# Ritesh622/Unbiased-Quantization-Distributed-Mean-Estimation

Hardware: AMD Instinct MI355X
Metric: quantize+dequantize M-vectors/sec at d=2^20 (1/2/4/8 GPU) + NMSE vs reference (higher is better)
Workload: dtype f32

## Files before the change

### include/uq_dme.h

```cpp
#ifndef UQ_DME_H
#define UQ_DME_H

#include <stddef.h>
#include <stdint.h>

#ifdef __cplusplus
extern "C" {
#endif

#define UQ_OK 0
#define UQ_E_INVALID (-1)
#define UQ_E_HIP (-2)
#define UQ_E_WORKSPACE (-3)
#define UQ_E_TIMEOUT (-4)

int uq_version(void);
const char* uq_build_id(void);
int uq_test_force_replay_failure(int on);
int uq_test_set_quicfl_hooks(int flags);
#define UQ_QFL_PLAN_FIELDS 6
#define UQ_QFL_SENDER 0
#define UQ_QFL_RECEIVER 1
#define UQ_QFL_FORM_NONE 0
#define UQ_QFL_FORM_ONE_WAVE 1
// ... 32 lines not shown
int uq_test_last_biased_plan(int64_t* plan_out, int32_t cap);
#define UQ_EDEN_PLAN_FIELDS 25
#define UQ_EDEN_NBITS_FRAC 12
#define UQ_EDEN_MAX_PASSES 4
#define UQ_EDEN_OP_COMPRESS 0
#define UQ_EDEN_OP_DECOMPRESS 1
#define UQ_EDEN_OP_RHT_FORWARD 2
#define UQ_EDEN_OP_RHT_INVERSE 3
#define UQ_EDEN_OP_NORM 4
#define UQ_EDEN_OP_QFL_FRONT 5
#define UQ_EDEN_OP_QFL_INVERSE 6
#define UQ_EDEN_OPS 7
#define UQ_EDEN_NORM_NONE 0
#define UQ_EDEN_NORM_CHAINS_WHOLE 1
#define UQ_EDEN_NORM_CHAINS_GENERIC 2
#define UQ_EDEN_NORM_SEGMENTED 3
#define UQ_EDEN_NORM_FUSED 4
#define UQ_EDEN_DOT_NONE 0
#define UQ_EDEN_DOT_ONE_WAVE 1
#define UQ_EDEN_DOT_SEGMENTED 2
#define UQ_EDEN_DOT_FUSED_REDO 3
#define UQ_EDEN_PASS_LOW16K 1
#define UQ_EDEN_PASS_LOW4096 2
#define UQ_EDEN_PASS_HIGH256 3
#define UQ_EDEN_PASS_SMALL 4
#define UQ_EDEN_PASS_GENERIC 5
int uq_test_eden_plan(int32_t op, int64_t n, int64_t dim, int32_t nbits, int32_t mode, int64_t* plan_out, int32_t cap);
int uq_test_last_eden_plan(int32_t op, int64_t* plan_out, int32_t cap);
#define UQ_EDEN_PACKED_PLAN_FIELDS 4
#define UQ_EDEN_PACKED_NONE 0
#define UQ_EDEN_PACKED_FUSED 1
#define UQ_EDEN_PACKED_CONVERTER 2
int uq_test_set_eden_hooks(int flags);
int uq_test_eden_packed_plan(int32_t op, int64_t n, int64_t dim, int32_t kind, int64_t* plan_out, int32_t cap);
int uq_test_last_eden_packed_plan(int32_t op, int64_t* plan_out, int32_t cap);
int uq_mt_jump_host(const uint32_t* state624, int64_t blocks, uint32_t* out624);

int uq_legacy_draw_f32(uint32_t* key624, int32_t* pos, int32_t* has_gauss, double* gauss, int32_t dist,
                       double a, double b, int64_t n, int64_t d, float* out, double* norm2, int32_t threads);
int uq_legacy_test_params(int64_t min_chunk, int64_t overlap, int64_t* waves, int64_t* misses);

const char* uq_last_error(void);

int uq_rate_to_m(double bits_per_dimension, int64_t d, int64_t* m_out);

int uq_workspace_bytes(int64_t n, int64_t d, int32_t torch_threads, size_t* bytes_out);

int uq_l1_torch_order_f32(const float* x, int64_t n, int64_t d, int32_t torch_threads,
                          float* l1_out, void* ws, size_t ws_bytes, void* stream);

int uq_type_unbiased_f32(const float* x, float* out, int64_t n, int64_t d, int64_t m,
                         const float* X, const float* l1, float* l1_out,
                         int32_t torch_threads, void* ws, size_t ws_bytes, void* stream);

int uq_type_unbiased_vec_f32(const float* x, float* out, int64_t d, int64_t m, float X, int32_t torch_threads,
                             void* ws, size_t ws_bytes, void* stream);

int uq_client_mean_f32(const float* q, int64_t n, int64_t d, int64_t ld, float n_div,
                       int32_t accumulate, float* est, void* stream);

int uq_type_unbiased_mean_f32(const float* x, float* out, int64_t n, int64_t d, int64_t m,
                              const float* X, const float* l1, int32_t torch_threads,
                              float n_div, int32_t accumulate, float* est,
                              void* ws, size_t ws_bytes, void* stream);

int uq_type_unbiased_codes_f32(const float* x, float* out, int8_t* codes, int32_t* kmax,
                               int64_t n, int64_t d, int64_t m, const float* X, const float* l1,
                               float* l1_out, int32_t torch_threads, void* ws, size_t ws_bytes,
                               void* stream);

int uq_type_unbiased_codes_ld_f32(const float* x, float* out, int64_t ldq, int8_t* codes, int64_t ldc,
                                  int32_t* kmax, int64_t n, int64_t d, int64_t m, const float* X,
                                  const float* l1, float* l1_out, int32_t torch_threads, void* ws,
                                  size_t ws_bytes, void* stream);

int uq_type_unbiased_nibbles_ld_f32(const float* x, float* out, int64_t ldq, uint8_t* nib, int64_t ldn,
                                    int32_t* kmax, int64_t n, int64_t d, int64_t m, const float* X,
                                    const float* l1, float* l1_out, int32_t torch_threads, void* ws,
                                    size_t ws_bytes, void* stream);

int uq_nibbles_q_mean_ld_f32(const uint8_t* nib, int64_t ldn, const float* q, int64_t ldq, const float* l1,
                             const int32_t* kmax, int64_t n, int64_t d, int64_t m, float n_div,
                             int32_t accumulate, float* est, void* stream);

int uq_codes_decode_f32(const int8_t* codes, const float* l1, int64_t n, int64_t d, int64_t m,
                        float* out, void* stream);

int uq_codes_mean_f32(const int8_t* codes, const float* l1, const int32_t* kmax, int64_t n, int64_t d,
                      int64_t m, float n_div, int32_t accumulate, float* est, void* stream);

int uq_codes_q_mean_f32(const int8_t* codes, const float* q, int64_t ldq, const float* l1, const int32_t* kmax,
                        int64_t n, int64_t d, int64_t m, float n_div, int32_t accumulate, float* est,
                        void* stream);

int uq_codes_q_mean_ld_f32(const int8_t* codes, int64_t ldc, const float* q, int64_t ldq, const float* l1,
                           const int32_t* kmax, int64_t n, int64_t d, int64_t m, float n_div,
                           int32_t accumulate, float* est, void* stream);

#define UQ_FORM_UNBIASED 0
#define UQ_FORM_BIASED 1
int uq_codes_decode_form_f32(const int8_t* codes, const float* l1, int64_t n, int64_t d, int64_t m, int32_t form,
                             float* out, void* stream);
int uq_codes_mean_form_f32(const int8_t* codes, int64_t ldc, const float* q, int64_t ldq, const float* l1,
                           const int32_t* kmax, int64_t n, int64_t d, int64_t m, int32_t form, float n_div,
                           int32_t accumulate, float* est, void* stream);

#define UQ_TC_EXACT_ZERO_SIGNS 1
#define UQ_TC_BIASED_FORM 2
int uq_tc_bound(int64_t d, size_t* bytes_out);
int uq_tc_workspace_bytes(int64_t n, int64_t d, size_t* bytes_out);
int uq_tc_encode(const int8_t* codes, const float* l1, int64_t n, int64_t d, int64_t m, int32_t flags,
                 uint8_t* msgs, size_t msgs_bytes, uint64_t* offsets, void* ws, size_t ws_bytes, void* stream);
int uq_tc_decode(const uint8_t* msgs, size_t msgs_bytes, const uint64_t* offsets, int64_t n, int64_t d, int64_t m,
                 int8_t* codes, float* l1, int32_t* kmax, int32_t* status, void* stream);

#define UQ_TIES_TORCH 0
#define UQ_TIES_LOWEST_INDEX 1
#define UQ_TIES_HOST_CHECK 4
int uq_biased_workspace_bytes(int64_t n, int64_t d, int32_t torch_threads, size_t* bytes_out);
int uq_type_biased_f32(const float* x, float* out, int64_t n, int64_t d, int64_t m,
                       int32_t torch_threads, int32_t tie_policy, float* l1_out, int32_t* info,
                       void* ws, size_t ws_bytes, void* stream);

int uq_biased_codes_workspace_bytes(int64_t n, int64_t d, int32_t torch_threads, size_t* bytes_out);
int uq_type_biased_codes_f32(const float* x, float* out, int8_t* codes, int32_t* kmax, int64_t n, int64_t d,
                             int64_t m, int32_t torch_threads, int32_t tie_policy, float* l1_out, int32_t* info,
                             void* ws, size_t ws_bytes, void* stream);

int uq_rht_signs(const int32_t* seeds, int64_t rows, int64_t D, int8_t* signs, void* stream);
int uq_rht_f32(const float* x, float* out, int64_t n, int64_t dim, int32_t inverse, const int8_t* signs,
               const int32_t* sign_row, void* ws, size_t ws_bytes, void* stream);
int uq_quicfl_prepare_f32(const int32_t* X, int64_t n, int64_t D, const float* recv_table, int32_t table_rows,
                          int32_t h_len, const int32_t* prng_seeds, const uint8_t* exact_mask, const float* exact_vals,
                          const float* scale, float* out, void* stream);
#define UQ_QFL_BAD_EXACT 32
int uq_quicfl_receive_f32(const void* X, int32_t x_kind, int64_t n, int64_t D, const float* recv_table,
                          int32_t table_rows, int32_t h_len, const int32_t* prng_seeds, const uint8_t* exact_mask,
                          const float* exact_vals, int32_t exact_layout, const int32_t* exact_count, const float* scale,
                          float* out, int32_t* info, void* stream);
int uq_quicfl_receive_workspace_bytes(int64_t n, int64_t D, size_t* bytes_out);
int uq_quicfl_receive_ws_f32(const void* X, int32_t x_kind, int64_t n, int64_t D, const float* recv_table,
                             int32_t table_rows, int32_t h_len, const int32_t* prng_seeds, const uint8_t* exact_mask,
                             const float* exact_vals, int32_t exact_layout, const int32_t* exact_count,
                             const float* scale, float* out, int32_t* info, void* ws, size_t ws_bytes, void* stream);

#define UQ_QFL_BAD_P 1
#define UQ_QFL_BAD_INDEX 2
#define UQ_QFL_BAD_PX 4
#define UQ_QFL_X_RANGE 8
#define UQ_QFL_TIMEOUT 16
#define UQ_QFL_STATE_WORDS 626
int uq_quicfl_workspace_bytes(int64_t n, int64_t dim, size_t* bytes_out);
int uq_quicfl_compress_f32(const float* x, int64_t n, int64_t dim, const int8_t* signs, const int32_t* sign_row,
                           const float* table_xp, const uint32_t* table_packed, int64_t table_numel, int32_t h_len,
                           float delta,
                           const int32_t* prng_seeds, const uint32_t* px_state, const int32_t* px_seeds,
                           uint32_t* px_state_out, void* X, int32_t x_kind, uint8_t* exact_mask, float* exact_vals,
                           int32_t* exact_count, float* scale, int32_t* info, void* ws, size_t ws_bytes, void* stream);
#define UQ_QFL_RECV_INDEX 64
int uq_quicfl_quantize_f32(const float* x, int64_t n, int64_t dim, const int8_t* signs, const int32_t* sign_row,
                           const float* table_xp, const uint32_t* table_packed, int64_t table_numel, int32_t h_len,
                           float delta, const float* recv_table, int32_t recv_numel, const int32_t* prng_seeds,
                           const uint32_t* px_state, const int32_t* px_seeds, uint32_t* px_state_out, float* out,
                           float* scale, int32_t* info, void* ws, size_t ws_bytes, void* stream);
int uq_test_set_quicfl_packed_hooks(int flags);
int uq_test_last_quicfl_packed_plan(int32_t side, int64_t* plan_out, int32_t cap);
// ... 101 lines not shown
```

### unbiased-quantization-distributed-mean-estimation_amd/_lib.py

```python
from __future__ import annotations

import ctypes
import os
import threading

from . import build_ext

_lock = threading.Lock()
_lib = None

_i32, _i64, _f32, _f64, _p, _sz = (ctypes.c_int32, ctypes.c_int64, ctypes.c_float,
                                   ctypes.c_double, ctypes.c_void_p, ctypes.c_size_t)
SIGNATURES = {
    "uq_version": (ctypes.c_int, []),
    "uq_last_error": (ctypes.c_char_p, []),
    "uq_build_id": (ctypes.c_char_p, []),
    "uq_test_force_replay_failure": (ctypes.c_int, [ctypes.c_int]),
    "uq_test_set_quicfl_hooks": (ctypes.c_int, [ctypes.c_int]),
    "uq_test_quicfl_plan": (ctypes.c_int, [_i32, _i64, _i64, _i32, _i32, _p, _i32]),
    "uq_test_last_quicfl_plan": (ctypes.c_int, [_i32, _p, _i32]),
    "uq_test_unbiased_plan": (ctypes.c_int, [_i64, _i64, _i64, _i64, _i32, _i32, _i32, _i32, _i32, _i32, _i32, _i32, _p,
                                             _i32]),
    "uq_test_last_unbiased_plan": (ctypes.c_int, [_p, _i32]),
    "uq_test_biased_plan": (ctypes.c_int, [_i64, _i64, _i32, _i32, _i32, _p, _i32]),
    "uq_test_last_biased_plan": (ctypes.c_int, [_p, _i32]),
    "uq_test_eden_plan": (ctypes.c_int, [_i32, _i64, _i64, _i32, _i32, _p, _i32]),
    "uq_test_last_eden_plan": (ctypes.c_int, [_i32, _p, _i32]),
    "uq_mt_jump_host": (ctypes.c_int, [_p, _i64, _p]),
    "uq_legacy_draw_f32": (ctypes.c_int, [_p, _p, _p, _p, _i32, _f64, _f64, _i64, _i64, _p, _p, _i32]),
    "uq_legacy_test_params": (ctypes.c_int, [_i64, _i64, _p, _p]),
    "uq_rate_to_m": (ctypes.c_int, [_f64, _i64, ctypes.POINTER(_i64)]),
    "uq_workspace_bytes": (ctypes.c_int, [_i64, _i64, _i32, ctypes.POINTER(_sz)]),
    "uq_l1_torch_order_f32": (ctypes.c_int, [_p, _i64, _i64, _i32, _p, _p, _sz, _p]),
    "uq_type_unbiased_f32": (ctypes.c_int, [_p, _p, _i64, _i64, _i64, _p, _p, _p, _i32, _p, _sz, _p]),
    "uq_type_unbiased_vec_f32": (ctypes.c_int, [_p, _p, _i64, _i64, _f32, _i32, _p, _sz, _p]),
    "uq_client_mean_f32": (ctypes.c_int, [_p, _i64, _i64, _i64, _f32, _i32, _p, _p]),
    "uq_type_unbiased_mean_f32": (ctypes.c_int, [_p, _p, _i64, _i64, _i64, _p, _p, _i32, _f32, _i32, _p,
                                                 _p, _sz, _p]),
    "uq_check_status": (ctypes.c_int, [_p, _p]),
    "uq_type_unbiased_codes_f32": (ctypes.c_int, [_p, _p, _p, _p, _i64, _i64, _i64, _p, _p, _p, _i32, _p, _sz, _p]),
    "uq_codes_decode_f32": (ctypes.c_int, [_p, _p, _i64, _i64, _i64, _p, _p]),
    "uq_codes_mean_f32": (ctypes.c_int, [_p, _p, _p, _i64, _i64, _i64, _f32, _i32, _p, _p]),
    "uq_codes_q_mean_f32": (ctypes.c_int, [_p, _p, _i64, _p, _p, _i64, _i64, _i64, _f32, _i32, _p, _p]),
    "uq_type_unbiased_codes_ld_f32": (ctypes.c_int, [_p, _p, _i64, _p, _i64, _p, _i64, _i64, _i64, _p, _p, _p, _i32,
                                                     _p, _sz, _p]),
    "uq_codes_q_mean_ld_f32": (ctypes.c_int, [_p, _i64, _p, _i64, _p, _p, _i64, _i64, _i64, _f32, _i32, _p, _p]),
    "uq_type_unbiased_nibbles_ld_f32": (ctypes.c_int, [_p, _p, _i64, _p, _i64, _p, _i64, _i64, _i64, _p, _p, _p, _i32,
                                                       _p, _sz, _p]),
    "uq_nibbles_q_mean_ld_f32": (ctypes.c_int, [_p, _i64, _p, _i64, _p, _p, _i64, _i64, _i64, _f32, _i32, _p, _p]),
    "uq_codes_decode_form_f32": (ctypes.c_int, [_p, _p, _i64, _i64, _i64, _i32, _p, _p]),
    "uq_codes_mean_form_f32": (ctypes.c_int, [_p, _i64, _p, _i64, _p, _p, _i64, _i64, _i64, _i32, _f32, _i32, _p, _p]),
    "uq_biased_codes_workspace_bytes": (ctypes.c_int, [_i64, _i64, _i32, ctypes.POINTER(_sz)]),
    "uq_type_biased_codes_f32": (ctypes.c_int, [_p, _p, _p, _p, _i64, _i64, _i64, _i32, _i32, _p, _p, _p, _sz, _p]),
    "uq_biased_workspace_bytes": (ctypes.c_int, [_i64, _i64, _i32, ctypes.POINTER(_sz)]),
    "uq_type_biased_f32": (ctypes.c_int, [_p, _p, _i64, _i64, _i64, _i32, _i32, _p, _p, _p, _sz, _p]),
    "uq_rht_signs": (ctypes.c_int, [_p, _i64, _i64, _p, _p]),
    "uq_rht_f32": (ctypes.c_int, [_p, _p, _i64, _i64, _i32, _p, _p, _p, _sz, _p]),
    "uq_quicfl_prepare_f32": (ctypes.c_int, [_p, _i64, _i64, _p, _i32, _i32, _p, _p, _p, _p, _p, _p]),
    "uq_quicfl_receive_f32": (ctypes.c_int, [_p, _i32, _i64, _i64, _p, _i32, _i32, _p, _p, _p, _i32, _p, _p, _p, _p, _p]),
    "uq_quicfl_receive_workspace_bytes": (ctypes.c_int, [_i64, _i64, ctypes.POINTER(_sz)]),
    "uq_quicfl_receive_ws_f32": (ctypes.c_int, [_p, _i32, _i64, _i64, _p, _i32, _i32, _p, _p, _p, _i32, _p, _p, _p, _p,
                                                _p, _sz, _p]),
    "uq_quicfl_workspace_bytes": (ctypes.c_int, [_i64, _i64, ctypes.POINTER(_sz)]),
    "uq_quicfl_quantize_f32": (ctypes.c_int, [_p, _i64, _i64, _p, _p, _p, _p, _i64, _i32, _f32, _p, _i32, _p, _p, _p, _p,
                                              _p, _p, _p, _p, _sz, _p]),
    "uq_quicfl_compress_f32": (ctypes.c_int, [_p, _i64, _i64, _p, _p, _p, _p, _i64, _i32, _f32, _p, _p, _p, _p, _p, _i32,
                                              _p, _p, _p, _p, _p, _p, _sz, _p]),
    "uq_test_set_quicfl_packed_hooks": (ctypes.c_int, [ctypes.c_int]),
    "uq_test_last_quicfl_packed_plan": (ctypes.c_int, [_i32, _p, _i32]),
    "uq_quicfl_packed_words": (ctypes.c_int, [_i64, _i32, ctypes.POINTER(_i64)]),
    "uq_quicfl_pack_x": (ctypes.c_int, [_p, _i32, _i64, _i64, _i32, _p, _p, _p, _p, _p, _p, _p]),
    "uq_quicfl_unpack_x": (ctypes.c_int, [_p, _i64, _i64, _i32, _p, _p, _p, _p, _p, _p]),
    "uq_quicfl_packed_workspace_bytes": (ctypes.c_int, [_i64, _i64, ctypes.POINTER(_sz)]),
    "uq_quicfl_compress_packed_f32": (ctypes.c_int, [_p, _i64, _i64, _p, _p, _p, _p, _i64, _i32, _f32, _p, _p, _p, _p, _p,
                                                     _i32, _p, _p, _p, _p, _p, _p, _p, _sz, _p]),
    "uq_quicfl_receive_packed_workspace_bytes": (ctypes.c_int, [_i64, _i64, ctypes.POINTER(_sz)]),
    "uq_quicfl_receive_packed_f32": (ctypes.c_int, [_p, _i32, _i64, _i64, _p, _i32, _i32, _p, _p, _p, _p, _p, _p, _p, _p,
                                                    _sz, _p]),
    "uq_xxh64": (ctypes.c_uint64, [ctypes.c_char_p, _sz, ctypes.c_uint64]),
    "uq_eden_workspace_bytes": (ctypes.c_int, [_i64, _i64, ctypes.POINTER(_sz)]),
    "uq_eden_compress_f32": (ctypes.c_int, [_p, _i64, _i64, _i32, _p, _p, _p, _p, _p, _sz, _p]),
    "uq_eden_decompress_f32": (ctypes.c_int, [_p, _p, _i64, _i64, _i32, _p, _p, _p, _p, _sz, _p]),
    "uq_eden_f32": (ctypes.c_int, [_p, _p, _i64, _i64, _i32, _p, _p, _p, _p, _sz, _p]),
    "uq_rht_sign_bits": (ctypes.c_int, [_p, _i64, _i64, _p, _p]),
    "uq_eden_compress_f32_sb": (ctypes.c_int, [_p, _i64, _i64, _i32, _p, _p, _p, _p, _p, _p, _sz, _p]),
    "uq_eden_decompress_f32_sb": (ctypes.c_int, [_p, _p, _i64, _i64, _i32, _p, _p, _p, _p, _p, _sz, _p]),
    "uq_eden_f32_sb": (ctypes.c_int, [_p, _p, _i64, _i64, _i32, _p, _p, _p, _p, _p, _sz, _p]),
    "uq_eden_mask_bits": (ctypes.c_int, [_p, _i64, _i64, ctypes.c_uint32, _p, _p]),
    "uq_eden_compress_frac_f32": (ctypes.c_int, [_p, _i64, _i64, _p, _p, _p, _p, _p, _p, _p, _p, _sz, _p]),
    "uq_eden_decompress_frac_f32": (ctypes.c_int, [_p, _p, _i64, _i64, _p, _p, _p, _p, _p, _p, _p, _sz, _p]),
    "uq_eden_frac_f32": (ctypes.c_int, [_p, _p, _i64, _i64, _p, _p, _p, _p, _p, _p, _p, _sz, _p]),
    "uq_test_set_eden_hooks": (ctypes.c_int, [ctypes.c_int]),
    "uq_test_eden_packed_plan": (ctypes.c_int, [_i32, _i64, _i64, _i32, _p, _i32]),
    "uq_test_last_eden_packed_plan": (ctypes.c_int, [_i32, _p, _i32]),
    "uq_eden_packed_words": (ctypes.c_int, [_i64, _i32, ctypes.POINTER(_i64)]),
    "uq_eden_packed_workspace_bytes": (ctypes.c_int, [_i64, _i64, _i32, ctypes.POINTER(_sz)]),
    "uq_eden_mask_ranks": (ctypes.c_int, [_p, _i64, _i64, _p, _p]),
    "uq_eden_pack_bins": (ctypes.c_int, [_p, _i64, _i64, _i32, _p, _p, _p, _p, _p, _p]),
    "uq_eden_unpack_bins": (ctypes.c_int, [_p, _i64, _i64, _i32, _p, _p, _p, _p, _p]),
    "uq_eden_compress_packed_f32": (ctypes.c_int, [_p, _i64, _i64, _i32, _p, _p, _p, _p, _p, _p, _p, _p, _p, _p, _sz, _p]),
    "uq_eden_decompress_packed_f32": (ctypes.c_int, [_p, _p, _i64, _i64, _i32, _p, _p, _p, _p, _p, _p, _p, _p, _sz, _p]),
    "uq_eden_norm_workspace_bytes": (ctypes.c_int, [_i64, _i64, ctypes.POINTER(_sz)]),
    "uq_eden_norm_f32": (ctypes.c_int, [_p, _i64, _i64, _i32, _p, _p, _sz, _p]),
    "uq_rand_workspace_bytes": (ctypes.c_int, [_i64, _i64, ctypes.POINTER(_sz)]),
    "uq_drive_words": (ctypes.c_int, [_i64, ctypes.POINTER(_i64)]),
    "uq_scalar_quantize_f32": (ctypes.c_int, [_p, _p, _i64, _i64, _f32, _p, _p, _p, _p, _p, _sz, _p]),
    "uq_drive_hadamard_f32": (ctypes.c_int, [_p, _p, _i64, _i64, _p, _p, _p, _p, _p, _sz, _p]),
    "uq_kashin_padded_dim": (ctypes.c_int, [_i64, ctypes.POINTER(_i64)]),
    "uq_kashin_workspace_bytes": (ctypes.c_int, [_i64, _i64, ctypes.POINTER(_sz)]),
    "uq_kashin_compress_f32": (ctypes.c_int, [_p, _i64, _i64, _i64, _i32, _f64, _f64, _f64, _i32, _p, _p, _p, _p, _i64,
                                              _p, _p, _p, _p, _p, _p, _sz, _p]),
    "uq_kashin_decompress_f32": (ctypes.c_int, [_p, _p, _p, _i64, _i64, _i64, _p, _p, _p, _p, _sz, _p]),
    "uq_kashin_f32": (ctypes.c_int, [_p, _p, _i64, _i64, _i64, _i32, _f64, _f64, _f64, _i32, _p, _p, _p, _p, _i64, _p, _p,
                                     _p, _p, _p, _sz, _p]),
    "uq_tc_bound":(ctypes.c_int, [_i64, ctypes.POINTER(_sz)]),
    "uq_tc_workspace_bytes": (ctypes.c_int, [_i64, _i64, ctypes.POINTER(_sz)]),
    "uq_tc_encode": (ctypes.c_int, [_p, _p, _i64, _i64, _i64, _i32, _p, _sz, _p, _p, _sz, _p]),
    "uq_tc_decode": (ctypes.c_int, [_p, _sz, _p, _i64, _i64, _i64, _p, _p, _p, _p, _p]),
}


class UQError(RuntimeError):
    """A C-ABI call returned a negative code."""


def library_path() -> str:
    return build_ext.SO


def load(build_if_missing: bool = False):
    global _lib
    with _lock:
# ... 25 lines not shown
```

### unbiased-quantization-distributed-mean-estimation_amd/csrc/uq_unbiased.hip

```cpp
#include <hip/hip_runtime.h>

#include <algorithm>
#include <cstdint>
#include <type_traits>

#include "uq_internal.h"
#include "uq_unbiased_kernels.h"

namespace {

struct WsLayout {
    size_t agg_off, incl_off, map1_off, rec_off, cnt_off, part_off, l1_off, total;
    int32_t tiles;
    template <class T>
    T* at(void* ws, size_t off) const { return (T*)((char*)ws + off); }
    uint64_t* tile_row(void* ws, size_t off, int64_t j0) const { return at<uint64_t>(ws, off) + j0 * tiles; }
};

WsLayout layout(int64_t n, int64_t d, const L1Plan& plan) {
    WsLayout w{};
    const int64_t tiles = (d + kQTile - 1) / kQTile;
    w.tiles = (int32_t)tiles;
    w.agg_off = kCtrlBytes;
    w.incl_off = up256(w.agg_off + (size_t)n * tiles * sizeof(uint64_t));
    w.map1_off = up256(w.incl_off + (size_t)n * tiles * sizeof(uint64_t));
    const size_t rec_clients = (size_t)std::min<int64_t>(n, kRecClients);
    w.rec_off = up256(w.map1_off + (size_t)n * tiles * sizeof(uint64_t));
    w.cnt_off = up256(w.rec_off + rec_clients * kRecPerClient * sizeof(TileRec));
    w.part_off = up256(w.cnt_off + rec_clients * sizeof(uint32_t));
    w.l1_off = up256(w.part_off + (size_t)n * plan.total_groups * 32 * sizeof(float));
    w.total = up256(w.l1_off + (size_t)n * sizeof(float));
    return w;
}

int launch_l1(const float* x, int64_t n, int64_t d, const L1Plan& plan, float* part, float* l1_out,
              hipStream_t st) {
    return launch_cascade<AbsOp>(x, n, d, plan, part, l1_out, nullptr, 0.f, st);
}

int stream_slots(int* out) {
    int dev = 0;
    int rc = hip_check(hipGetDevice(&dev), "hipGetDevice");
    if (rc) return rc;
    static thread_local int cache_dev = -1, cache_slots = 0;
    if (cache_dev != dev) {
        int cus = 0;
        rc = hip_check(hipDeviceGetAttribute(&cus, hipDeviceAttributeMultiprocessorCount, dev), "CU count");
        if (rc) return rc;
        cache_slots = 4 * std::max(1, cus);
        cache_dev = dev;
    }
    *out = cache_slots;
    return UQ_OK;
}

int check_common(const void* x, int64_t n, int64_t d, int32_t T, void* ws, size_t ws_bytes,
                 L1Plan* plan, WsLayout* w) {
    if (n < 0 || d < 0) return fail(UQ_E_INVALID, "n and d must be >= 0");
    if (n > (int64_t)1 << 31 || d > (int64_t)1 << 40) return fail(UQ_E_INVALID, "n or d too large");
    if (T < 1) return fail(UQ_E_INVALID, "torch_threads must be >= 1");
    if (!make_plan(d, T, plan)) return fail(UQ_E_INVALID, "torch_threads > 4096 (or d too large) unsupported by the L1 plan");
    *w = layout(n, d, *plan);
    if ((int64_t)w->tiles * n > 0xFFFFFFFFll) return fail(UQ_E_INVALID, "batch too large for one call");
    if (n > 0 && d > 0) {
        if (!x) return fail(UQ_E_INVALID, "null input pointer");
        if (!ws) return fail(UQ_E_INVALID, "null workspace");
        if (ws_bytes < w->total) return fail(UQ_E_WORKSPACE, "workspace too small");
    }
    return UQ_OK;
}

}

int uq_internal::launch_l1(const float* x, int64_t n, int64_t d, int32_t T, float* part, float* l1_out,
                           hipStream_t st) {
    L1Plan plan;
    if (!make_plan(d, T, &plan)) return fail(UQ_E_INVALID, "cannot build L1 plan");
    return ::launch_l1(x, n, d, plan, part, l1_out, st);
}

extern "C" {

int uq_workspace_bytes(int64_t n, int64_t d, int32_t T, size_t* bytes_out) {
    if (!bytes_out) return fail(UQ_E_INVALID, "null bytes_out");
    L1Plan plan;
// ... 57 lines not shown
    int32_t prefixed, R, nseg;
};
struct UnbiasedPlan {
    int32_t form;
    bool V, Q, C, CV, l1_given;
    int64_t chunks;
    ChunkPlan last;
    int32_t tiles;
    size_t agg_off, map0_off, map1_off, rec_off, cnt_off;
};

int chunk_plan(const PlanIn& in, const UnbiasedPlan& p, int64_t j0, ChunkPlan* c) {
    c->nj = std::min<int64_t>(kMaxGridY, in.n - j0);
    const int64_t total_tiles = c->nj * (int64_t)p.tiles;
    c->seg = p.V && in.d <= ((int64_t)1 << 29) && total_tiles >= kSegMinTiles;
    c->R = 1;
    c->nseg = 1;
    if (c->seg) {
        int slots = in.slots;
        if (slots <= 0) {
            const int rc = stream_slots(&slots);
            if (rc) return rc;
        }
        const int64_t segs = std::max<int64_t>(1, slots / c->nj);
        c->R = (int32_t)((p.tiles + segs - 1) / segs);
        c->nseg = (p.tiles + c->R - 1) / c->R;
    }
    c->prefixed = c->nj >= 4 ? 1 : 0;
    return UQ_OK;
}

int plan_unbiased(const PlanIn& in, const WsLayout& w, UnbiasedPlan* p) {
    *p = UnbiasedPlan{};
    if (!in.has_out && !in.has_codes) return fail(UQ_E_INVALID, "nothing to write: out and codes are both NULL");
    const int64_t n = in.n, d = in.d;
    p->tiles = w.tiles;
    p->agg_off = w.agg_off;
    p->map0_off = w.incl_off;
    p->map1_off = w.map1_off;
    p->rec_off = w.rec_off;
    p->cnt_off = w.cnt_off;
    p->Q = in.has_out;
    p->C = in.has_codes;
    p->l1_given = in.l1_given;
    p->V = in.x16 && (!in.has_out || in.out16) && ((d % 4 == 0 && in.ldo % 4 == 0) || n == 1);
    p->CV = !in.has_codes || (in.codes16 && d % 16 == 0 && (in.ldc % 16 == 0 || n == 1));
    p->chunks = 1;
    p->last = ChunkPlan{n, false, 0, w.tiles, 1};
    if (!in.nib && d <= kSmallL1Max && p->V && n <= 0x7FFFFFFF) {
        p->form = UQ_FORM_SMALL;
        return UQ_OK;
    }
    const bool stream_form = n >= kStreamMinClients && p->V && d <= ((int64_t)1 << 29);
    if (in.nib) {
        if (!stream_form || !in.has_out || !in.has_codes)
            return fail(UQ_E_INVALID, "internal: 4-bit codes outside the stream form");
        p->form = UQ_FORM_STREAM_NIBBLES;
        p->CV = true;
        return UQ_OK;
    }
    if (stream_form) {
        p->form = UQ_FORM_STREAM;
        return UQ_OK;
    }
    p->chunks = (n + kMaxGridY - 1) / kMaxGridY;
    const int rc = chunk_plan(in, *p, (p->chunks - 1) * kMaxGridY, &p->last);
    if (rc) return rc;
    p->form = p->last.seg ? UQ_FORM_SEGMENTS : UQ_FORM_PHASED;
    return UQ_OK;
}

bool bad_pitches(bool has_out, int64_t ldo, bool has_codes, int64_t ldc, int64_t d, bool nib) {
    return (has_out && ldo < d) || (has_codes && ldc < (nib ? d / 2 : d));
}

bool bad_nibble_shape(int64_t n, int64_t d) {
    return n < kStreamMinClients || d % kNibAlign != 0 || d > ((int64_t)1 << 29);
}
int nibble_shape_error() {
    return fail(UQ_E_INVALID, "4-bit codes need n >= 256 and d a multiple of 4096 (<= 2^29)");
}

thread_local UnbiasedPlan t_last_plan{};

int export_plan(const UnbiasedPlan& p, int64_t* out, int32_t cap) {
    if (!out || cap < 0) return fail(UQ_E_INVALID, "null plan output");
    const int64_t f[UQ_PLAN_FIELDS] = {
        p.form, p.V, p.Q, p.C, p.CV, p.l1_given, p.chunks, p.last.nj, p.last.prefixed, p.last.R, p.last.nseg,
        p.tiles, (int64_t)p.agg_off, (int64_t)p.map0_off, (int64_t)p.map1_off, (int64_t)p.rec_off, (int64_t)p.cnt_off,
        (int64_t)sizeof(TileRec), kRecPerClient, kRecClients, kRecEvents, kFoldEvents};
    for (int i = 0; i < std::min<int32_t>(cap, UQ_PLAN_FIELDS); ++i) out[i] = f[i];
    return UQ_OK;
}

int unbiased_codes_impl(const float* x, float* out, int64_t ldo, int8_t* codes, int64_t ldc, int32_t* overflow,
                        int64_t n, int64_t d, int64_t m, const float* X, float Xval, const float* l1, float* l1_out,
                        int32_t T, void* ws, size_t ws_bytes, void* stream, bool nib = false) {
    L1Plan plan;
    WsLayout w;
    int rc = check_common(x, n, d, T, ws, ws_bytes, &plan, &w);
    if (rc) return rc;
    t_last_plan = UnbiasedPlan{};
    if (m < 0) return fail(UQ_E_INVALID, "m must be >= 0");
    if (bad_pitches(out, ldo, codes, ldc, d, nib)) return fail(UQ_E_INVALID, "row pitches must be >= d");
    if (n == 0 || d == 0) return UQ_OK;
    if (!X && n != 1) return fail(UQ_E_INVALID, "null X");
    const PlanIn in{n, d, ldo, ldc, aligned16(x), aligned16(out), aligned16(codes), out != nullptr, codes != nullptr,
                    nib, l1 != nullptr, 0};
    UnbiasedPlan P;
    rc = plan_unbiased(in, w, &P);
    if (rc) return rc;
    if (codes && !overflow) return fail(UQ_E_INVALID, "codes need a kmax[n] array");
    t_last_plan = P;
    hipStream_t st = (hipStream_t)stream;
    const float* l1use = l1;
    const float fm = (float)m;
    const bool vec4 = P.V, cvec = P.CV;
    if (P.form == UQ_FORM_SMALL) {
        if (!select_qc(out, codes, cvec, [&](auto Q, auto C, auto CV) {
                hipLaunchKernelGGL((quantize_small_kernel<Q(), C(), CV()>), dim3((unsigned)n), dim3(kQBlock), 0, st, x,
                                   out, codes, overflow, d, w.tiles, fm, X, Xval, l1, l1_out, ldo, ldc);
            }))
            return bad_selector();
        return hip_check(hipGetLastError(), "quantize_small_kernel launch");
    }
    if (!l1use) {
        float* l1buf = w.at<float>(ws, w.l1_off);
        rc = launch_l1(x, n, d, plan, w.at<float>(ws, w.part_off), l1buf, st);
        if (rc) return rc;
        l1use = l1buf;
    }
    if (l1_out && l1_out != l1use) {
        rc = hip_check(hipMemcpyAsync(l1_out, l1use, n * sizeof(float), hipMemcpyDeviceToDevice, st), "copy l1");
        if (rc) return rc;
    }
    const bool stream_form = P.form == UQ_FORM_STREAM || P.form == UQ_FORM_STREAM_NIBBLES;
    if (codes && !stream_form) {
        rc = hip_check(hipMemsetAsync(overflow, 0, n * sizeof(int32_t), st), "memset kmax");
        if (rc) return rc;
    }
    if (P.form == UQ_FORM_STREAM_NIBBLES) {
        hipLaunchKernelGGL((quantize_stream_kernel<true, true, true, true>), dim3((unsigned)n), dim3(kQBlock), 0, st, x,
                           out, codes, overflow, d, w.tiles, fm, X, Xval, l1use, w.tiles, 1, nullptr, ldo, ldc);
        return hip_check(hipGetLastError(), "quantize_stream_kernel (4-bit codes) launch");
    }
    if (P.form == UQ_FORM_STREAM) {
        if (!select_qc(out, codes, cvec, [&](auto Q, auto C, auto CV) {
                hipLaunchKernelGGL((quantize_stream_kernel<Q(), C(), CV()>), dim3((unsigned)n), dim3(kQBlock), 0, st, x,
                                   out, codes, overflow, d, w.tiles, fm, X, Xval, l1use, w.tiles, 1, nullptr, ldo, ldc);
            }))
            return bad_selector();
        return hip_check(hipGetLastError(), "quantize_stream_kernel launch");
    }
    for (int64_t j0 = 0; j0 < n; j0 += kMaxGridY) {
        ChunkPlan ck;
        rc = chunk_plan(in, P, j0, &ck);
        if (rc) return rc;
        const int64_t nj = ck.nj;
        const float* xj = x + j0 * d;
        float* outj = out ? out + j0 * ldo : nullptr;
        int8_t* codesj = codes ? codes + j0 * ldc : nullptr;
        int32_t* ovj = codes ? overflow + j0 : nullptr;
        const float* Xj = X ? X + j0 : nullptr;
        const float* l1j = l1use + j0;
        uint64_t* agg = w.tile_row(ws, w.agg_off, j0);
        uint64_t* pre = w.tile_row(ws, w.incl_off, j0);
// ... 10 lines not shown
            hipLaunchKernelGGL(tile_agg_kernel<true>, tgrid, dim3(kQBlock), 0, st, xj, d, w.tiles, fm, l1j, agg, reccnt);
        } else {
            hipLaunchKernelGGL(tile_agg_kernel<false>, tgrid, dim3(kQBlock), 0, st, xj, d, w.tiles, fm, l1j, agg, reccnt);
        }
        rc = hip_check(hipGetLastError(), "tile sums launch");
        if (rc) return rc;
        const int32_t prefixed = ck.prefixed;
        if (prefixed) {
            hipLaunchKernelGGL(tile_prefix_kernel, dim3((unsigned)nj), dim3(kQBlock), 0, st, agg, w.tiles);
            rc = hip_check(hipGetLastError(), "tile_prefix_kernel launch");
            if (rc) return rc;
        }
        const auto map_and_fold = [&](auto V) {
            hipLaunchKernelGGL((tile_map_kernel<V()>), tgrid, dim3(kQBlock), 0, st, xj, d, w.tiles, fm, l1j, agg, pre, map1,
                               recs, reccnt, prefixed);
            const int e = hip_check(hipGetLastError(), "tile_map_kernel launch");
            if (e) return e;
            hipLaunchKernelGGL((exact_fold_kernel<V()>), dim3((unsigned)nj), dim3(kQBlock), 0, st, xj, d, w.tiles, fm, l1j,
                               pre, map1, agg, recs, reccnt);
            return hip_check(hipGetLastError(), "exact_fold_kernel launch");
        };
        rc = vec4 ? map_and_fold(Flag<true>{}) : map_and_fold(Flag<false>{});
        if (rc) return rc;
        pre = agg;
        if (seg) {
            if (!select_qc(out, codes, cvec, [&](auto Q, auto C, auto CV) {
                    hipLaunchKernelGGL((quantize_stream_kernel<Q(), C(), CV()>), dim3((unsigned)(nj * nseg)),
                                       dim3(kQBlock), 0, st, xj, outj, codesj, ovj, d, w.tiles, fm, Xj, Xval, l1j, R, nseg,
                                       pre, ldo, ldc);
                }))
                return bad_selector();
            rc = hip_check(hipGetLastError(), "quantize_stream_kernel (segments) launch");
            if (rc) return rc;
            continue;
        }
        if (!select_vqc(vec4, out, codes, cvec, [&](auto V, auto Q, auto C, auto CV) {
                hipLaunchKernelGGL((tile_out_kernel<V(), Q(), C(), CV()>), tgrid, dim3(kQBlock), 0, st, xj, outj, codesj,
                                   ovj, d, w.tiles, fm, Xj, Xval, l1j, pre, ldo, ldc);
            }))
            return bad_selector();
        rc = hip_check(hipGetLastError(), "tile_out_kernel launch");
        if (rc) return rc;
    }
    return UQ_OK;
}

}

extern "C" {

int uq_type_unbiased_codes_ld_f32(const float* x, float* out, int64_t ldq, int8_t* codes, int64_t ldc,
                                  int32_t* overflow, int64_t n, int64_t d, int64_t m, const float* X, const float* l1,
                                  float* l1_out, int32_t T, void* ws, size_t ws_bytes, void* stream) {
    if (n > 0 && d > 0 && !X) return fail(UQ_E_INVALID, "null X");
    return unbiased_codes_impl(x, out, ldq, codes, ldc, overflow, n, d, m, X, 0.0f, l1, l1_out, T, ws, ws_bytes,
                               stream);
}

int uq_type_unbiased_nibbles_ld_f32(const float* x, float* out, int64_t ldq, uint8_t* nib, int64_t ldn,
                                    int32_t* kmax, int64_t n, int64_t d, int64_t m, const float* X, const float* l1,
                                    float* l1_out, int32_t T, void* ws, size_t ws_bytes, void* stream) {
    if (n < 0 || d < 0) return fail(UQ_E_INVALID, "n and d must be >= 0");
    if (n == 0 || d == 0) return UQ_OK;
    if (!x || !out || !nib || !kmax || !X) return fail(UQ_E_INVALID, "null pointer (x, out, codes, kmax and X are required)");
    if (bad_nibble_shape(n, d)) return nibble_shape_error();
    if (ldq < d || ldq % 4 != 0 || ldn < d / 2 || ldn % 16 != 0 || !aligned16(x) || !aligned16(out) || !aligned16(nib))
        return fail(UQ_E_INVALID, "4-bit codes need 16-byte aligned rows: ldq >= d, ldq % 4 == 0, ldn >= d/2, ldn % 16 == 0");
    return unbiased_codes_impl(x, out, ldq, (int8_t*)nib, ldn, kmax, n, d, m, X, 0.0f, l1, l1_out, T, ws, ws_bytes,
                               stream, true);
}

int uq_nibbles_q_mean_ld_f32(const uint8_t* nib, int64_t ldn, const float* q, int64_t ldq, const float* l1,
                             const int32_t* kmax, int64_t n, int64_t d, int64_t m, float n_div, int32_t accumulate,
                             float* est, void* stream) {
    if (n < 0 || d < 0 || m < 0) return fail(UQ_E_INVALID, "n, d and m must be >= 0");
    if (d == 0) return UQ_OK;
    if (!est || (n > 0 && (!nib || !l1 || !kmax || !q))) return fail(UQ_E_INVALID, "null pointer (q is required)");
    if (d % kNibAlign != 0 || ldq < d || ldq % 4 != 0 || ldn < d / 2 || ldn % 4 != 0 || !aligned16(est) ||
        (n > 0 && (!aligned16(q) || ((uintptr_t)nib & 3u))))
        return fail(UQ_E_INVALID, "4-bit code mean: d % 4096 == 0, ldq >= d (multiple of 4), ldn >= d/2 (multiple of 4), "
                                  "16-byte aligned est and q");
    const int64_t blocks = d / (kCodesMeanThreads * kMeanCpt);
    if (blocks > 0x7FFFFFFF) return fail(UQ_E_INVALID, "d too large");
    hipLaunchKernelGGL(nibbles_mean_kernel, dim3((unsigned)blocks), dim3(kCodesMeanThreads), 0, (hipStream_t)stream, nib,
                       ldn, l1, kmax, n, d, (float)m, n_div, accumulate, est, q, ldq);
    return hip_check(hipGetLastError(), "nibbles_mean_kernel launch");
}

int uq_type_unbiased_codes_f32(const float* x, float* out, int8_t* codes, int32_t* overflow, int64_t n, int64_t d,
                               int64_t m, const float* X, const float* l1, float* l1_out, int32_t T, void* ws,
                               size_t ws_bytes, void* stream) {
    return uq_type_unbiased_codes_ld_f32(x, out, d, codes, d, overflow, n, d, m, X, l1, l1_out, T, ws, ws_bytes,
                                         stream);
}

int uq_type_unbiased_vec_f32(const float* x, float* out, int64_t d, int64_t m, float X, int32_t T, void* ws,
                             size_t ws_bytes, void* stream) {
    if (d > 0 && !out) return fail(UQ_E_INVALID, "null out");
    return unbiased_codes_impl(x, out, d, nullptr, d, nullptr, 1, d, m, nullptr, X, nullptr, nullptr, T, ws, ws_bytes,
                               stream);
}

int uq_type_unbiased_f32(const float* x, float* out, int64_t n, int64_t d, int64_t m, const float* X,
                         const float* l1, float* l1_out, int32_t T, void* ws, size_t ws_bytes,
                         void* stream) {
    if (n > 0 && d > 0 && !out) return fail(UQ_E_INVALID, "null out");
    return uq_type_unbiased_codes_f32(x, out, nullptr, nullptr, n, d, m, X, l1, l1_out, T, ws, ws_bytes, stream);
}

int uq_codes_decode_f32(const int8_t* codes, const float* l1, int64_t n, int64_t d, int64_t m, float* out,
                        void* stream) {
    return uq_codes_decode_form_f32(codes, l1, n, d, m, UQ_FORM_UNBIASED, out, stream);
}

int uq_codes_decode_form_f32(const int8_t* codes, const float* l1, int64_t n, int64_t d, int64_t m, int32_t form,
                             float* out, void* stream) {
    if (n < 0 || d < 0 || m < 0) return fail(UQ_E_INVALID, "n, d and m must be >= 0");
    if (form != UQ_FORM_UNBIASED && form != UQ_FORM_BIASED) return fail(UQ_E_INVALID, "unknown codes form");
    if (form == UQ_FORM_BIASED && m < 1) return fail(UQ_E_INVALID, "m must be >= 1 for biased codes");
    if (n == 0 || d == 0) return UQ_OK;
    if (!codes || !l1 || !out) return fail(UQ_E_INVALID, "null pointer");
    hipStream_t st = (hipStream_t)stream;
    const int64_t chunks = (d + kDecChunk - 1) / kDecChunk;
    if (chunks > 0x7FFFFFFF) return fail(UQ_E_INVALID, "d too large");
    const bool vec = aligned16(codes) && aligned16(out) && d % 16 == 0;
    dim3 grid((unsigned)chunks, (unsigned)n);
    if (form == UQ_FORM_BIASED) {
        if (vec)
            hipLaunchKernelGGL(codes_decode_biased_kernel<true>, grid, dim3(256), 0, st, codes, l1, d, (float)m, out);
        else
            hipLaunchKernelGGL(codes_decode_biased_kernel<false>, grid, dim3(256), 0, st, codes, l1, d, (float)m, out);
    } else if (vec)
        hipLaunchKernelGGL(codes_decode_kernel<true>, grid, dim3(256), 0, st, codes, l1, d, (float)m, out);
    else
        hipLaunchKernelGGL(codes_decode_kernel<false>, grid, dim3(256), 0, st, codes, l1, d, (float)m, out);
    return hip_check(hipGetLastError(), "codes_decode_kernel launch");
}

int uq_codes_q_mean_ld_f32(const int8_t* codes, int64_t ldc, const float* q, int64_t ldq, const float* l1,
                           const int32_t* kmax, int64_t n, int64_t d, int64_t m, float n_div, int32_t accumulate,
                           float* est, void* stream) {
    return uq_codes_mean_form_f32(codes, ldc, q, ldq, l1, kmax, n, d, m, UQ_FORM_UNBIASED, n_div, accumulate, est, stream);
}

int uq_codes_mean_form_f32(const int8_t* codes, int64_t ldc, const float* q, int64_t ldq, const float* l1,
                           const int32_t* kmax, int64_t n, int64_t d, int64_t m, int32_t form, float n_div,
                           int32_t accumulate, float* est, void* stream) {
    if (n < 0 || d < 0 || m < 0) return fail(UQ_E_INVALID, "n, d and m must be >= 0");
    if (form != UQ_FORM_UNBIASED && form != UQ_FORM_BIASED) return fail(UQ_E_INVALID, "unknown codes form");
    if (form == UQ_FORM_BIASED && m < 1) return fail(UQ_E_INVALID, "m must be >= 1 for biased codes");
    if (d == 0) return UQ_OK;
    if (!est || (n > 0 && (!codes || !l1 || !kmax))) return fail(UQ_E_INVALID, "null pointer");
    if (q && ldq < d) return fail(UQ_E_INVALID, "ldq must be >= d");
    if (ldc < d) return fail(UQ_E_INVALID, "ldc must be >= d");
    hipStream_t st = (hipStream_t)stream;
    const bool vec = (n == 0 || aligned16(codes)) && aligned16(est) && d % 16 == 0 && ldc % 16 == 0;
    const int64_t blocks = (d + kCodesMeanThreads * kMeanCpt - 1) / (kCodesMeanThreads * kMeanCpt);
    if (blocks > 0x7FFFFFFF) return fail(UQ_E_INVALID, "d too large");
    const dim3 tb(kCodesMeanThreads);
    if (form == UQ_FORM_BIASED) {
        if (vec && d % (kCodesMeanThreads * kMeanCpt) == 0)
            hipLaunchKernelGGL((codes_mean_biased_kernel<true, true>), dim3((unsigned)blocks), tb, 0, st, codes, ldc, l1, kmax,
                               n, d, (float)m, n_div, accumulate, est, q, ldq);
        else if (vec)
            hipLaunchKernelGGL(codes_mean_biased_kernel<true>, dim3((unsigned)blocks), tb, 0, st, codes, ldc, l1, kmax, n, d,
                               (float)m, n_div, accumulate, est, q, ldq);
        else
            hipLaunchKernelGGL(codes_mean_biased_kernel<false>, dim3((unsigned)blocks), tb, 0, st, codes, ldc, l1, kmax, n, d,
                               (float)m, n_div, accumulate, est, q, ldq);
// ... 76 lines not shown
```

### unbiased-quantization-distributed-mean-estimation_amd/csrc/uq_unbiased_kernels.h

```cpp

#ifndef UQ_UNBIASED_KERNELS_H
#define UQ_UNBIASED_KERNELS_H

#include "uq_common.h"

namespace {

constexpr int kQItems = 16;
constexpr int kQTile = kQBlock * kQItems;
constexpr int64_t kStreamMinClients = 256;
constexpr int64_t kSegMinTiles = 1024;

struct AbsOp {
    static constexpr bool kHist = false;
    float den, fm;
    uint32_t *h, *zn;
    __device__ static AbsOp make(const float*, float, int64_t) { return AbsOp{0.f, 0.f, nullptr, nullptr}; }
    __device__ float operator()(float v) const { return fabsf(v); }
    __device__ void apply4(const float (&v)[4], float (&a)[4]) const {
#pragma unroll
        for (int c = 0; c < 4; ++c) a[c] += fabsf(v[c]);
    }
};

// ... 1410 lines not shown
        const float* tb = tab[jj + u];
#pragma unroll
        for (int k = 0; k < kMeanCpt; ++k) e[k] += tb[(w[u] >> (4 * k)) & 0xFu];
    }
}

constexpr int kNibChunk = 1024;
__device__ __forceinline__ void nib_build_tables(float (*tab)[16], const float* __restrict__ l1,
                                                 const int32_t* __restrict__ kmaxv, int64_t j0, int nb, float fm,
                                                 float n_div) {
    for (int e = threadIdx.x; e < nb * 8; e += kCodesMeanThreads) {
        const int jj = e >> 3, k = e & 7;
        const float L = l1[j0 + jj];
        const int km = min(kNibMax, max(0, kmaxv[j0 + jj]));
        if (k <= km) {
            const float v = ((L * (float)k) / fm) / n_div;
            tab[jj][k] = v;
            tab[jj][15 - k] = -v;
        }
    }
}

__global__ void __launch_bounds__(kCodesMeanThreads)
nibbles_mean_kernel(const uint8_t* __restrict__ nib, int64_t ldn, const float* __restrict__ l1,
                    const int32_t* __restrict__ kmaxv, int64_t n, int64_t d, float fm, float n_div, int accumulate,
                    float* __restrict__ est, const float* __restrict__ q, int64_t ldq) {
    __shared__ float tab[kNibChunk][16];
    __shared__ uint32_t s_ovf;
    const int tid = threadIdx.x;
    const int64_t i0 = ((int64_t)blockIdx.x * kCodesMeanThreads + tid) * kMeanCpt;
    float e[kMeanCpt];
    if (accumulate) {
        const float4 a = *reinterpret_cast<const float4*>(est + i0), b = *reinterpret_cast<const float4*>(est + i0 + 4);
        e[0] = a.x; e[1] = a.y; e[2] = a.z; e[3] = a.w; e[4] = b.x; e[5] = b.y; e[6] = b.z; e[7] = b.w;
    } else {
#pragma unroll
        for (int k = 0; k < kMeanCpt; ++k) e[k] = 0.0f;
    }
    if (tid == 0) s_ovf = 0u;
    __syncthreads();
    bool a = false;
    for (int64_t j = tid; j < n; j += kCodesMeanThreads) a = a || kmaxv[j] > kNibMax;
    if (a) s_ovf = 1u;
    __syncthreads();
    const bool any = s_ovf != 0u;
    const uint8_t* cbase = nib + i0 / 2;
    for (int64_t c0 = 0; c0 < n; c0 += kNibChunk) {
        const int nc = (int)min((int64_t)kNibChunk, n - c0);
        __syncthreads();
        nib_build_tables(tab, l1, kmaxv, c0, nc, fm, n_div);
        __syncthreads();
        const int full = any ? 0 : nc / kMeanClients * kMeanClients;
        if (full > 0) {
            uint32_t wa[kMeanUnroll], wb[kMeanUnroll];
            const uint8_t* cb = cbase + c0 * ldn;
            nib_load_batch(wa, cb, ldn);
            for (int g = 0; g < full; g += kMeanClients) {
                nib_load_batch(wb, cb + (int64_t)(g + kMeanUnroll) * ldn, ldn);
                nib_add_batch(e, wa, tab, g);
                const int gn = (g + kMeanClients + kMeanUnroll <= nc) ? g + kMeanClients : nc - kMeanUnroll;
                nib_load_batch(wa, cb + (int64_t)gn * ldn, ldn);
                nib_add_batch(e, wb, tab, g + kMeanUnroll);
            }
        }
        for (int jj = full; jj < nc; ++jj) {
            const int64_t j = c0 + jj;
            if (kmaxv[j] > kNibMax) {
                const float4 a4 = *reinterpret_cast<const float4*>(q + j * ldq + i0);
                const float4 b4 = *reinterpret_cast<const float4*>(q + j * ldq + i0 + 4);
                const float qq[kMeanCpt] = {a4.x, a4.y, a4.z, a4.w, b4.x, b4.y, b4.z, b4.w};
#pragma unroll
                for (int k = 0; k < kMeanCpt; ++k) e[k] += qq[k] / n_div;
            } else {
                const uint32_t w = *reinterpret_cast<const uint32_t*>(cbase + j * ldn);
#pragma unroll
                for (int k = 0; k < kMeanCpt; ++k) e[k] += tab[jj][(w >> (4 * k)) & 0xFu];
            }
        }
    }
    *reinterpret_cast<float4*>(est + i0) = make_float4(e[0], e[1], e[2], e[3]);
    *reinterpret_cast<float4*>(est + i0 + 4) = make_float4(e[4], e[5], e[6], e[7]);
}

}

#endif
```

Before: 0.4290.

## Add pair-table nibble mean kernel for small-magnitude codes

Adds a new nibble-mean kernel. When every client's kmax fits within a small range, it builds per-client 64-entry pair lookup tables in LDS and decodes two nibbles per LDS load, using SDWA byte-select shifts to compute the offsets. This halves the LDS lookups and the per-nibble extraction work in the mean accumulation. Otherwise it falls back to the original 16-entry table path. It adds a per-block scan of kmax, writes a device-global path flag, and adds a test hook to force the old kernel.

Result: faster. 0.4335, median of 6 (+1.1%).

```diff
diff --git a/include/uq_dme.h b/include/uq_dme.h
--- a/include/uq_dme.h
+++ b/include/uq_dme.h
@@ -138,6 +138,11 @@
 int uq_nibbles_q_mean_ld_f32(const uint8_t* nib, int64_t ldn, const float* q, int64_t ldq, const float* l1,
                              const int32_t* kmax, int64_t n, int64_t d, int64_t m, float n_div,
                              int32_t accumulate, float* est, void* stream);
+#define UQ_NIB_PATH_PAIRS 1
+#define UQ_NIB_PATH_TABLES 2
+#define UQ_NIB_PATH_MIXED 3
+int uq_test_nibble_mean_path(void* stream, int32_t* path_out);
+int uq_test_set_nibble_mean_hooks(int flags);
 
 int uq_codes_decode_f32(const int8_t* codes, const float* l1, int64_t n, int64_t d, int64_t m,
                         float* out, void* stream);
diff --git a/unbiased-quantization-distributed-mean-estimation_amd/_lib.py b/unbiased-quantization-distributed-mean-estimation_amd/_lib.py
--- a/unbiased-quantization-distributed-mean-estimation_amd/_lib.py
+++ b/unbiased-quantization-distributed-mean-estimation_amd/_lib.py
@@ -48,6 +48,8 @@
     "uq_type_unbiased_nibbles_ld_f32": (ctypes.c_int, [_p, _p, _i64, _p, _i64, _p, _i64, _i64, _i64, _p, _p, _p, _i32,
                                                        _p, _sz, _p]),
     "uq_nibbles_q_mean_ld_f32": (ctypes.c_int, [_p, _i64, _p, _i64, _p, _p, _i64, _i64, _i64, _f32, _i32, _p, _p]),
+    "uq_test_nibble_mean_path": (ctypes.c_int, [_p, _p]),
+    "uq_test_set_nibble_mean_hooks": (ctypes.c_int, [ctypes.c_int]),
     "uq_codes_decode_form_f32": (ctypes.c_int, [_p, _p, _i64, _i64, _i64, _i32, _p, _p]),
     "uq_codes_mean_form_f32": (ctypes.c_int, [_p, _i64, _p, _i64, _p, _p, _i64, _i64, _i64, _i32, _f32, _i32, _p, _p]),
     "uq_biased_codes_workspace_bytes": (ctypes.c_int, [_i64, _i64, _i32, ctypes.POINTER(_sz)]),
diff --git a/unbiased-quantization-distributed-mean-estimation_amd/csrc/uq_unbiased.hip b/unbiased-quantization-distributed-mean-estimation_amd/csrc/uq_unbiased.hip
--- a/unbiased-quantization-distributed-mean-estimation_amd/csrc/uq_unbiased.hip
+++ b/unbiased-quantization-distributed-mean-estimation_amd/csrc/uq_unbiased.hip
@@ -1,6 +1,7 @@
 #include <hip/hip_runtime.h>
 
 #include <algorithm>
+#include <atomic>
 #include <cstdint>
 #include <type_traits>
 
@@ -224,6 +225,7 @@
 }
 
 thread_local UnbiasedPlan t_last_plan{};
+std::atomic<int> g_nib_mean_hooks{0};
 
 int export_plan(const UnbiasedPlan& p, int64_t* out, int32_t cap) {
     if (!out || cap < 0) return fail(UQ_E_INVALID, "null plan output");
@@ -400,9 +402,26 @@
                                   "16-byte aligned est and q");
     const int64_t blocks = d / (kCodesMeanThreads * kMeanCpt);
     if (blocks > 0x7FFFFFFF) return fail(UQ_E_INVALID, "d too large");
-    hipLaunchKernelGGL(nibbles_mean_kernel, dim3((unsigned)blocks), dim3(kCodesMeanThreads), 0, (hipStream_t)stream, nib,
-                       ldn, l1, kmax, n, d, (float)m, n_div, accumulate, est, q, ldq);
-    return hip_check(hipGetLastError(), "nibbles_mean_kernel launch");
+    if (g_nib_mean_hooks.load(std::memory_order_relaxed) & 1) {
+        hipLaunchKernelGGL(nibbles_mean_kernel, dim3((unsigned)blocks), dim3(kCodesMeanThreads), 0, (hipStream_t)stream,
+                           nib, ldn, l1, kmax, n, d, (float)m, n_div, accumulate, est, q, ldq);
+        return hip_check(hipGetLastError(), "nibbles_mean_kernel launch");
+    }
+    hipLaunchKernelGGL(nibbles_mean_pairs_kernel, dim3((unsigned)blocks), dim3(kCodesMeanThreads), 0, (hipStream_t)stream,
+                       nib, ldn, l1, kmax, n, d, (float)m, n_div, accumulate, est, q, ldq);
+    return hip_check(hipGetLastError(), "nibbles_mean_pairs_kernel launch");
+}
+
+int uq_test_set_nibble_mean_hooks(int flags) { return g_nib_mean_hooks.exchange(flags); }
+
+int uq_test_nibble_mean_path(void* stream, int32_t* path_out) {
+    if (!path_out) return fail(UQ_E_INVALID, "null path_out");
+    int rc = hip_check(hipStreamSynchronize((hipStream_t)stream), "nibble mean path: synchronize");
+    if (rc) return rc;
+    const int32_t zero = 0;
+    rc = hip_check(hipMemcpyFromSymbol(path_out, HIP_SYMBOL(g_nib_mean_path), sizeof(int32_t)), "nibble mean path: read");
+    if (rc) return rc;
+    return hip_check(hipMemcpyToSymbol(HIP_SYMBOL(g_nib_mean_path), &zero, sizeof(int32_t)), "nibble mean path: clear");
 }
 
 int uq_type_unbiased_codes_f32(const float* x, float* out, int8_t* codes, int32_t* overflow, int64_t n, int64_t d,
diff --git a/unbiased-quantization-distributed-mean-estimation_amd/csrc/uq_unbiased_kernels.h b/unbiased-quantization-distributed-mean-estimation_amd/csrc/uq_unbiased_kernels.h
--- a/unbiased-quantization-distributed-mean-estimation_amd/csrc/uq_unbiased_kernels.h
+++ b/unbiased-quantization-distributed-mean-estimation_amd/csrc/uq_unbiased_kernels.h
@@ -1516,6 +1516,163 @@
     *reinterpret_cast<float4*>(est + i0 + 4) = make_float4(e[4], e[5], e[6], e[7]);
 }
 
+constexpr int kPairMax = 3;
+constexpr int kPairChunk = 128;
+constexpr int kPairBytes = 512;
+static_assert(kPairChunk % kMeanClients == 0 && (kPairChunk - 1) * kPairBytes + 63 * 8 < 65536,
+              "whole code groups per chunk, client bases within 16 bits");
+static_assert(kPairChunk == kMeanUnroll * (kCodesMeanThreads / kWave), "pair_build_tables: 16 clients per wave");
+
+__device__ int32_t g_nib_mean_path;
+
+__device__ __forceinline__ void pair_build_tables(unsigned char* ptab, float L, float fm, float n_div, int wid, int lane) {
+    const float v = ((L * (float)(lane & 3)) / fm) / n_div;
+    const int lo = lane & 7, hi = lane >> 3;
+    const int slo = lo < 4 ? lo : 7 - lo, shi = hi < 4 ? hi : 7 - hi;
+    const uint32_t nlo = lo < 4 ? 0u : 0x80000000u, nhi = hi < 4 ? 0u : 0x80000000u;
+    unsigned char* dst = ptab + (wid * kMeanUnroll) * kPairBytes + lane * 8;
+#pragma unroll
+    for (int c = 0; c < kMeanUnroll; ++c) {
+        const uint32_t a = __float_as_uint(__shfl(v, 4 * c + slo)) ^ nlo;
+        const uint32_t b = __float_as_uint(__shfl(v, 4 * c + shi)) ^ nhi;
+        *reinterpret_cast<uint2*>(dst + c * kPairBytes) = make_uint2(a, b);
+    }
+}
+
+template <int B>
+__device__ __forceinline__ uint32_t pair_offset(uint32_t c, uint32_t three) {
+    uint32_t a;
+    if (B == 0) asm("v_lshlrev_b32_sdwa %0, %1, %2 dst_sel:DWORD dst_unused:UNUSED_PAD src0_sel:DWORD src1_sel:BYTE_0" : "=v"(a) : "v"(three), "v"(c));
+    if (B == 1) asm("v_lshlrev_b32_sdwa %0, %1, %2 dst_sel:DWORD dst_unused:UNUSED_PAD src0_sel:DWORD src1_sel:BYTE_1" : "=v"(a) : "v"(three), "v"(c));
+    if (B == 2) asm("v_lshlrev_b32_sdwa %0, %1, %2 dst_sel:DWORD dst_unused:UNUSED_PAD src0_sel:DWORD src1_sel:BYTE_2" : "=v"(a) : "v"(three), "v"(c));
+    if (B == 3) asm("v_lshlrev_b32_sdwa %0, %1, %2 dst_sel:DWORD dst_unused:UNUSED_PAD src0_sel:DWORD src1_sel:BYTE_3" : "=v"(a) : "v"(three), "v"(c));
+    return a;
+}
+
+__device__ __forceinline__ void pair_add_word(float (&e)[kMeanCpt], uint32_t w, const unsigned char* tb) {
+    const uint32_t c = (w & 0x07070707u) | ((w >> 1) & 0x38383838u);
+    const uint32_t o[4] = {pair_offset<0>(c, 3u), pair_offset<1>(c, 3u), pair_offset<2>(c, 3u), pair_offset<3>(c, 3u)};
+#pragma unroll
+    for (int b = 0; b < 4; ++b) {
+        const float2 v = *reinterpret_cast<const float2*>(tb + o[b]);
+        e[2 * b] += v.x;
+        e[2 * b + 1] += v.y;
+    }
+}
+
+__device__ __forceinline__ void pair_add_batch(float (&e)[kMeanCpt], const uint32_t (&w)[kMeanUnroll], const unsigned char* tb) {
+#pragma unroll
+    for (int u = 0; u < kMeanUnroll; ++u) pair_add_word(e, w[u], tb + u * kPairBytes);
+}
+
+__global__ void __launch_bounds__(kCodesMeanThreads)
+nibbles_mean_pairs_kernel(const uint8_t* __restrict__ nib, int64_t ldn, const float* __restrict__ l1,
+                          const int32_t* __restrict__ kmaxv, int64_t n, int64_t d, float fm, float n_div,
+                          int accumulate, float* __restrict__ est, const float* __restrict__ q, int64_t ldq) {
+    __shared__ float tab[kNibChunk][16];
+    __shared__ uint32_t s_ovf;
+    const int tid = threadIdx.x;
+    const int64_t i0 = ((int64_t)blockIdx.x * kCodesMeanThreads + tid) * kMeanCpt;
+    float e[kMeanCpt];
+    if (accumulate) {
+        const float4 a = *reinterpret_cast<const float4*>(est + i0), b = *reinterpret_cast<const float4*>(est + i0 + 4);
+        e[0] = a.x; e[1] = a.y; e[2] = a.z; e[3] = a.w; e[4] = b.x; e[5] = b.y; e[6] = b.z; e[7] = b.w;
+    } else {
+#pragma unroll
+        for (int k = 0; k < kMeanCpt; ++k) e[k] = 0.0f;
+    }
+    if (tid == 0) s_ovf = 0u;
+    __syncthreads();
+    bool a = false, p = false;
+    for (int64_t j = tid; j < n; j += kCodesMeanThreads) {
+        a = a || kmaxv[j] > kNibMax;
+        p = p || kmaxv[j] > kPairMax;
+    }
+    if (p) atomicOr(&s_ovf, a ? 3u : 2u);
+    __syncthreads();
+    const bool any = (s_ovf & 1u) != 0u;
+    const uint8_t* cbase = nib + i0 / 2;
+    const bool pairs = s_ovf == 0u;
+    if (blockIdx.x == 0 && tid == 0) g_nib_mean_path = pairs ? UQ_NIB_PATH_PAIRS : any ? UQ_NIB_PATH_MIXED : UQ_NIB_PATH_TABLES;
+    if (pairs) {
+        static_assert(sizeof(tab) == kPairChunk * kPairBytes, "a chunk's pair tables take the LDS of the 16-entry tables");
+        unsigned char* ptab = reinterpret_cast<unsigned char*>(&tab[0][0]);
+        const int lane = tid & (kWave - 1);
+        const int wid = __builtin_amdgcn_readfirstlane(tid / kWave);
+        const int64_t jl = wid * kMeanUnroll + (lane >> 2);
+        float L = n > 0 ? l1[min(jl, n - 1)] : 0.0f;
+        uint32_t wa[kMeanUnroll], wb[kMeanUnroll];
+        if (n >= kMeanClients) nib_load_batch(wa, cbase, ldn);
+        for (int64_t c0 = 0; c0 < n; c0 += kPairChunk) {
+            const int nc = (int)min((int64_t)kPairChunk, n - c0);
+            __syncthreads();
+            pair_build_tables(ptab, L, fm, n_div, wid, lane);
+            L = l1[min(c0 + kPairChunk + jl, n - 1)];
+            __syncthreads();
+            const uint8_t* cb = cbase + c0 * ldn;
+            if (nc == kPairChunk) {
+#pragma unroll
+                for (int g = 0; g < kPairChunk; g += kMeanClients) {
+                    nib_load_batch(wb, cb + (int64_t)(g + kMeanUnroll) * ldn, ldn);
+                    pair_add_batch(e, wa, ptab + g * kPairBytes);
+                    const int64_t jn = (c0 + g + kMeanClients + kMeanUnroll <= n) ? c0 + g + kMeanClients : n - kMeanUnroll;
+                    nib_load_batch(wa, cbase + jn * ldn, ldn);
+                    pair_add_batch(e, wb, ptab + (g + kMeanUnroll) * kPairBytes);
+                }
+            } else {
+                const int full = nc / kMeanClients * kMeanClients;
+                for (int g = 0; g < full; g += kMeanClients) {
+                    nib_load_batch(wb, cb + (int64_t)(g + kMeanUnroll) * ldn, ldn);
+                    pair_add_batch(e, wa, ptab + g * kPairBytes);
+                    const int64_t jn = (c0 + g + kMeanClients + kMeanUnroll <= n) ? c0 + g + kMeanClients : n - kMeanUnroll;
+                    nib_load_batch(wa, cbase + jn * ldn, ldn);
+                    pair_add_batch(e, wb, ptab + (g + kMeanUnroll) * kPairBytes);
+                }
+                for (int jj = full; jj < nc; ++jj)
+                    pair_add_word(e, *reinterpret_cast<const uint32_t*>(cb + (int64_t)jj * ldn), ptab + jj * kPairBytes);
+            }
+        }
+        *reinterpret_cast<float4*>(est + i0) = make_float4(e[0], e[1], e[2], e[3]);
+        *reinterpret_cast<float4*>(est + i0 + 4) = make_float4(e[4], e[5], e[6], e[7]);
+        return;
+    }
+    for (int64_t c0 = 0; c0 < n; c0 += kNibChunk) {
+        const int nc = (int)min((int64_t)kNibChunk, n - c0);
+        __syncthreads();
+        nib_build_tables(tab, l1, kmaxv, c0, nc, fm, n_div);
+        __syncthreads();
+        const int full = any ? 0 : nc / kMeanClients * kMeanClients;
+        if (full > 0) {
+            uint32_t wa[kMeanUnroll], wb[kMeanUnroll];
+            const uint8_t* cb = cbase + c0 * ldn;
+            nib_load_batch(wa, cb, ldn);
+            for (int g = 0; g < full; g += kMeanClients) {
+                nib_load_batch(wb, cb + (int64_t)(g + kMeanUnroll) * ldn, ldn);
+                nib_add_batch(e, wa, tab, g);
+                const int gn = (g + kMeanClients + kMeanUnroll <= nc) ? g + kMeanClients : nc - kMeanUnroll;
+                nib_load_batch(wa, cb + (int64_t)gn * ldn, ldn);
+                nib_add_batch(e, wb, tab, g + kMeanUnroll);
+            }
+        }
+        for (int jj = full; jj < nc; ++jj) {
+            const int64_t j = c0 + jj;
+            if (kmaxv[j] > kNibMax) {
+                const float4 a4 = *reinterpret_cast<const float4*>(q + j * ldq + i0);
+                const float4 b4 = *reinterpret_cast<const float4*>(q + j * ldq + i0 + 4);
+                const float qq[kMeanCpt] = {a4.x, a4.y, a4.z, a4.w, b4.x, b4.y, b4.z, b4.w};
+#pragma unroll
+                for (int k = 0; k < kMeanCpt; ++k) e[k] += qq[k] / n_div;
+            } else {
+                const uint32_t w = *reinterpret_cast<const uint32_t*>(cbase + j * ldn);
+#pragma unroll
+                for (int k = 0; k < kMeanCpt; ++k) e[k] += tab[jj][(w >> (4 * k)) & 0xFu];
+            }
+        }
+    }
+    *reinterpret_cast<float4*>(est + i0) = make_float4(e[0], e[1], e[2], e[3]);
+    *reinterpret_cast<float4*>(est + i0 + 4) = make_float4(e[4], e[5], e[6], e[7]);
+}
+
 }
 
 #endif
```
